# fabiocarrara/neural-ode-features

Measured on AMD Instinct MI355X. Metric: images/sec (fwd+adjoint) CIFAR-10 ODE-ResNet bs=128 at 1/2/4/8 GPU, higher is better.
Workload: dtype f32

## Files before the change

### neural-ode-features_amd/csrc/kernels_stem.hip

```cpp
#include "stem.h"

namespace node {

namespace {

typedef float f32x16 __attribute__((ext_vector_type(16)));
typedef __bf16 bf16x8 __attribute__((ext_vector_type(8)));
typedef __bf16 bf16x2 __attribute__((ext_vector_type(2)));
typedef float f32x2 __attribute__((ext_vector_type(2)));
typedef unsigned u32x4 __attribute__((ext_vector_type(4)));

__device__ __forceinline__ void split3(float x, bf16_t& h, bf16_t& m, bf16_t& l) {
  const __bf16 bh = (__bf16)x;
  const float r = x - (float)bh;
  const __bf16 bm = (__bf16)r;
  const float r2 = r - (float)bm;
  const __bf16 bl = (__bf16)r2;
  h = __builtin_bit_cast(bf16_t, bh);
  m = __builtin_bit_cast(bf16_t, bm);
  l = __builtin_bit_cast(bf16_t, bl);
}
__device__ __forceinline__ void split8(const float4& p, const float4& q, u32x4& hh, u32x4& mm, u32x4& ll) {
  const f32x2 v[4] = {{p.x, p.y}, {p.z, p.w}, {q.x, q.y}, {q.z, q.w}};
#pragma unroll
  for (int i = 0; i < 4; ++i) {
    const bf16x2 h = __builtin_convertvector(v[i], bf16x2);
    const f32x2 r = v[i] - __builtin_convertvector(h, f32x2);
    const bf16x2 m = __builtin_convertvector(r, bf16x2);
    const f32x2 r2 = r - __builtin_convertvector(m, f32x2);
    const bf16x2 l = __builtin_convertvector(r2, bf16x2);
    hh[i] = __builtin_bit_cast(unsigned, h);
    mm[i] = __builtin_bit_cast(unsigned, m);
    ll[i] = __builtin_bit_cast(unsigned, l);
  }
}
__device__ __forceinline__ float bf16_f(bf16_t v) { return __builtin_bit_cast(float, (unsigned)v << 16); }

typedef __attribute__((address_space(3))) void* lds_ptr_t;
typedef short s16x4 __attribute__((ext_vector_type(4)));
__device__ __forceinline__ int img_off(int row, int piece) { return row * 128 + ((piece ^ ((row >> 1) & 7)) << 4); }
__device__ __forceinline__ void glds16(const bf16_t* src, unsigned char* lds_dst) {
  __builtin_amdgcn_global_load_lds(reinterpret_cast<const void*>(src), (lds_ptr_t)lds_dst, 16, 0, 0);
}

__global__ __launch_bounds__(256) void k_stem_conv(const SConvArgs a) {
  constexpr int BM = 128, BN = 64;
  constexpr int A_PLANE = BM * 128, B_PLANE = BN * 128, A_BYTES = 3 * A_PLANE, BUF = A_BYTES + 3 * B_PLANE;
  extern __shared__ __align__(16) unsigned char smem[];
  int* out_off = reinterpret_cast<int*>(smem + 2 * BUF);
  const int t = threadIdx.x, lane = t & 63, wave = __builtin_amdgcn_readfirstlane(t >> 6);
  const int ntn = a.Cout / BN;
  int b = blockIdx.x;
  const int nblk = gridDim.x;
  if ((nblk & 7) == 0) b = (b & 7) * (nblk >> 3) + (b >> 3);
  const int ntn_all = (a.mode == 0 && a.w2 != nullptr) ? 2 * ntn : ntn;
  const int tile_m = b / ntn_all;
  int tile_n = b - tile_m * ntn_all;
  const bool shortcut_tile = tile_n >= ntn;
  if (shortcut_tile) tile_n -= ntn;
  int tile0 = 0, ch = a.cls_h[0], cw = a.cls_w[0], cpy = a.cls_py[0], cpx = a.cls_px[0], ntap = a.cls_ntap[0];
  unsigned long long taps = a.cls_taps[0];
#pragma unroll
  for (int c = 1; c < 4; ++c)
    if (c < a.nclass && tile_m >= a.cls_tile0[c]) {
      tile0 = a.cls_tile0[c]; ch = a.cls_h[c]; cw = a.cls_w[c]; cpy = a.cls_py[c]; cpx = a.cls_px[c]; ntap = a.cls_ntap[c];
      taps = a.cls_taps[c];
    }
  if (shortcut_tile) { ntap = 1; taps = (unsigned long long)((a.KH >> 1) * a.KW + (a.KW >> 1)); }
  const bf16_t* wsel = shortcut_tile ? a.w2 : a.w;
  const size_t wsel_plane = shortcut_tile ? a.w2_plane : a.w_plane;
  const int wtaps_one = shortcut_tile ? 1 : 0;
  const bool extra_k = a.mode == 1 && a.in2 != nullptr && cpy == 0 && cpx == 0 && a.step == 2;
  const int row0 = (tile_m - tile0) * BM;
  const int Mc = a.N * ch * cw;
  const int lrow = lane >> 3, lslot = lane & 7;
  int rn[4], roy[4], rox[4];
  bool rval[4];
#pragma unroll
  for (int j = 0; j < 4; ++j) {
    const int rl = 32 * wave + 8 * j + lrow, r = row0 + rl;
    rval[j] = r < Mc;
    rn[j] = roy[j] = rox[j] = 0;
    if (rval[j]) {
      rn[j] = r / (ch * cw);
      const int rem = r - rn[j] * ch * cw;
      const int cy = rem / cw;
      roy[j] = cy * a.step + cpy;
      rox[j] = (rem - cy * cw) * a.step + cpx;
    }
    if (lslot == 0) out_off[rl] = rval[j] ? (rn[j] * a.OH + roy[j]) * a.OW + rox[j] : -1;
  }
  const int ncc = a.Cin >> 6;
  const int nmain = ntap * ncc;
  const int nchunk = nmain + (extra_k ? ncc : 0);

  auto issue = [&](int q, int buf) {
    unsigned char* A = smem + buf * BUF;
    unsigned char* B = A + A_BYTES;
    const bool xk = q >= nmain;
    const int qq = xk ? q - nmain : q;
    const int ti = qq / ncc, c0 = (qq - ti * ncc) << 6;
    const int tap = xk ? 0 : (int)((taps >> (4 * ti)) & 15);
    const int ky = xk ? 0 : tap / a.KW, kx = xk ? 0 : tap - ky * a.KW;
    const int pad = xk ? 0 : a.pad;
    const bf16_t* in = xk ? a.in2 : a.in;
    const bf16_t* wq = xk ? a.w2 : wsel;
    const size_t wq_plane = xk ? a.w2_plane : wsel_plane;
    const int wtap = (xk || wtaps_one) ? 0 : tap;
#pragma unroll
    for (int j = 0; j < 4; ++j) {
      int iy, ix;
      bool ok = rval[j];
      if (a.mode == 0) {
        iy = (roy[j] << a.sshift) + ky - pad;
        ix = (rox[j] << a.sshift) + kx - pad;
      } else {
        const int ty = roy[j] + pad - ky, tx = rox[j] + pad - kx;
        ok = ok && ty >= 0 && tx >= 0;
        iy = ty >> a.sshift;
        ix = tx >> a.sshift;
      }
      ok = ok && (unsigned)iy < (unsigned)a.IH && (unsigned)ix < (unsigned)a.IW;
      const int irow = ok ? (rn[j] * a.IH + iy) * a.IW + ix : a.zero_row;
      const int rl = 32 * wave + 8 * j + lrow;
      const bf16_t* src = in + (size_t)irow * a.Cin + c0 + ((lslot ^ ((rl >> 1) & 7)) << 3);
#pragma unroll
      for (int p = 0; p < 3; ++p) glds16(src + p * a.in_plane, A + p * A_PLANE + (32 * wave + 8 * j) * 128);
    }
#pragma unroll
    for (int j = 0; j < 2; ++j) {
      const int col = 16 * wave + 8 * j + lrow;
      const bf16_t* ws = wq + ((size_t)wtap * a.Cout + tile_n * BN + col) * a.Cin + c0 + ((lslot ^ ((col >> 1) & 7)) << 3);
#pragma unroll
      for (int p = 0; p < 3; ++p) glds16(ws + p * wq_plane, B + p * B_PLANE + (16 * wave + 8 * j) * 128);
    }
  };

  f32x16 acc[2];
#pragma unroll
  for (int c = 0; c < 2; ++c)
#pragma unroll
    for (int i = 0; i < 16; ++i) acc[c][i] = 0.f;

  issue(0, 0);
  const int li = lane & 31, lg = lane >> 5;
  const int arow = 32 * wave + li;
  for (int q = 0; q < nchunk; ++q) {
    __syncthreads();
    if (q + 1 < nchunk) issue(q + 1, (q + 1) & 1);
    const unsigned char* A = smem + (q & 1) * BUF;
    const unsigned char* B = A + A_BYTES;
#pragma unroll
    for (int ks = 0; ks < 4; ++ks) {
      bf16x8 fa[3];
#pragma unroll
      for (int p = 0; p < 3; ++p)
        fa[p] = __builtin_bit_cast(bf16x8, *reinterpret_cast<const u32x4*>(A + p * A_PLANE + img_off(arow, 2 * ks + lg)));
#pragma unroll
      for (int c = 0; c < 2; ++c) {
        const int brow = 32 * c + li;
        bf16x8 fb[3];
#pragma unroll
        for (int p = 0; p < 3; ++p)
          fb[p] = __builtin_bit_cast(bf16x8, *reinterpret_cast<const u32x4*>(B + p * B_PLANE + img_off(brow, 2 * ks + lg)));
        acc[c] = __builtin_amdgcn_mfma_f32_32x32x16_bf16(fa[2], fb[0], acc[c], 0, 0, 0);
        acc[c] = __builtin_amdgcn_mfma_f32_32x32x16_bf16(fa[0], fb[2], acc[c], 0, 0, 0);
        acc[c] = __builtin_amdgcn_mfma_f32_32x32x16_bf16(fa[1], fb[1], acc[c], 0, 0, 0);
        acc[c] = __builtin_amdgcn_mfma_f32_32x32x16_bf16(fa[1], fb[0], acc[c], 0, 0, 0);
        acc[c] = __builtin_amdgcn_mfma_f32_32x32x16_bf16(fa[0], fb[1], acc[c], 0, 0, 0);
        acc[c] = __builtin_amdgcn_mfma_f32_32x32x16_bf16(fa[0], fb[0], acc[c], 0, 0, 0);
      }
    }
  }

#pragma unroll
  for (int c = 0; c < 2; ++c) {
    const int col = tile_n * BN + 32 * c + li;
    const float bv = a.bias ? a.bias[col] : 0.f;
#pragma unroll
    for (int i = 0; i < 16; ++i) {
      const int rl = 32 * wave + 8 * (i >> 2) + 4 * lg + (i & 3);
      const int off = out_off[rl];
      if (off < 0) continue;
      const size_t o = (size_t)off * a.Cout + col;
      if (shortcut_tile) { a.out2[o] = acc[c][i]; continue; }
      float v = acc[c][i] + bv;
      if (a.res) v += a.res[o];
      if (a.accumulate) v += a.out[o];
      a.out[o] = v;
    }
  }
}

template <int TG, bool EXTRA>
__global__ __launch_bounds__(256) void k_stem_wgrad(const SWgradArgs a) {
  constexpr int IMG = 3 * 16 * 128;
  constexpr int NIMG = 1 + TG + (EXTRA ? 1 : 0);
  constexpr int BUF = NIMG * IMG;
  extern __shared__ __align__(16) unsigned char smem[];
  const int t = threadIdx.x, lane = t & 63, wave = __builtin_amdgcn_readfirstlane(t >> 6);
  const int nct = a.Cin >> 6, npair = nct * (a.Cout >> 6);
  const int ngrp = TG == 3 ? 3 : 1;
  int bb = blockIdx.x;
  const int pair = bb % npair; bb /= npair;
  const int ky = bb % ngrp;
  const int split = bb / ngrp;
  const int cot = pair / nct, cit = pair - cot * nct;
  const bool extra = EXTRA && ky == 1;
  const int rows = a.N * a.OH * a.OW;
  const int rbeg = split * a.rows_per_split;
  const int rend = min(rbeg + a.rows_per_split, rows);
  const int nchunk = rbeg < rend ? (rend - rbeg + 15) >> 4 : 0;

  const int lrow = lane >> 3, lslot = lane & 7;
  int pn[2], py[2], px[2];
#pragma unroll
  for (int h = 0; h < 2; ++h) {
    const int r = rbeg + 8 * h + lrow;
    pn[h] = r / (a.OH * a.OW);
    const int rem = r - pn[h] * a.OH * a.OW;
    py[h] = rem / a.OW;
    px[h] = rem - py[h] * a.OW;
  }
  auto issue = [&](int q, int buf) {
    unsigned char* base = smem + buf * BUF;
    const int r0 = rbeg + 16 * q;
    constexpr int NINST = NIMG * 6;
#pragma unroll
    for (int ii = 0; ii < (NINST + 3) / 4; ++ii) {
      const int inst = wave + 4 * ii;
      if (inst >= NINST) break;
      const int im = inst / 6, part = (inst % 6) >> 1, h = inst & 1;
      if (EXTRA && !extra && im == NIMG - 1) continue;
      const int rl = 8 * h + lrow;
      const bool valid = r0 + rl < rend;
      const int sw = (lslot ^ ((rl >> 1) & 7)) << 3;
      const bf16_t* src;
      if (im == 0 || (EXTRA && im == NIMG - 1)) {
        const bf16_t* d = im == 0 ? a.dy3 : a.dy23;
        src = d + part * a.dy_plane + (size_t)(valid ? r0 + rl : a.dy_zero_row) * a.Cout + cot * 64 + sw;
      } else {
        const int kx = TG == 3 ? im - 1 : 0;
        const int iy = py[h] * a.stride - a.pad + (TG == 3 ? ky : 0), ix = px[h] * a.stride - a.pad + kx;
        const bool ok = valid && (unsigned)iy < (unsigned)a.IH && (unsigned)ix < (unsigned)a.IW;
        src = a.in + part * a.in_plane + (size_t)(ok ? (pn[h] * a.IH + iy) * a.IW + ix : a.zero_row) * a.Cin + cit * 64 + sw;
      }
      glds16(src, base + im * IMG + part * 2048 + h * 1024);
    }
#pragma unroll
    for (int h = 0; h < 2; ++h) {
      px[h] += 16;
      while (px[h] >= a.OW) { px[h] -= a.OW; py[h] += 1; }
      while (py[h] >= a.OH) { py[h] -= a.OH; pn[h] += 1; }
    }
  };

  constexpr int NA = TG + (EXTRA ? 1 : 0);
  f32x16 acc[NA];
#pragma unroll
  for (int j = 0; j < NA; ++j)
#pragma unroll
    for (int i = 0; i < 16; ++i) acc[j][i] = 0.f;

  const int cob = wave >> 1, cib = wave & 1;
  const int kg = lane >> 5, g16 = (lane >> 4) & 1, m = lane & 15, tq = m >> 2, tp = m & 3;
  auto frag = [&](const unsigned char* img, int part, int cb0) -> bf16x8 {
    const int piece = ((cb0 + 16 * g16) >> 3) + (tp >> 1), inb = (tp & 1) << 3;
    const int r0 = 8 * kg + tq, r1 = r0 + 4;
    const s16x4 lo = __builtin_amdgcn_ds_read_tr16_b64_v4i16((__attribute__((address_space(3))) s16x4*)(img + part * 2048 + img_off(r0, piece) + inb));
    const s16x4 hi = __builtin_amdgcn_ds_read_tr16_b64_v4i16((__attribute__((address_space(3))) s16x4*)(img + part * 2048 + img_off(r1, piece) + inb));
    typedef short s16x8 __attribute__((ext_vector_type(8)));
    const s16x8 v = {lo[0], lo[1], lo[2], lo[3], hi[0], hi[1], hi[2], hi[3]};
    return __builtin_bit_cast(bf16x8, v);
  };

  if (nchunk > 0) issue(0, 0);
  for (int q = 0; q < nchunk; ++q) {
    __syncthreads();
    if (q + 1 < nchunk) issue(q + 1, (q + 1) & 1);
    const unsigned char* base = smem + (q & 1) * BUF;
    bf16x8 fa[3];
#pragma unroll
    for (int p = 0; p < 3; ++p) fa[p] = frag(base, p, 32 * cob);
#pragma unroll
    for (int j = 0; j < TG; ++j) {
      bf16x8 fb[3];
#pragma unroll
      for (int p = 0; p < 3; ++p) fb[p] = frag(base + (1 + j) * IMG, p, 32 * cib);
      acc[j] = __builtin_amdgcn_mfma_f32_32x32x16_bf16(fa[2], fb[0], acc[j], 0, 0, 0);
      acc[j] = __builtin_amdgcn_mfma_f32_32x32x16_bf16(fa[0], fb[2], acc[j], 0, 0, 0);
      acc[j] = __builtin_amdgcn_mfma_f32_32x32x16_bf16(fa[1], fb[1], acc[j], 0, 0, 0);
      acc[j] = __builtin_amdgcn_mfma_f32_32x32x16_bf16(fa[1], fb[0], acc[j], 0, 0, 0);
      acc[j] = __builtin_amdgcn_mfma_f32_32x32x16_bf16(fa[0], fb[1], acc[j], 0, 0, 0);
      acc[j] = __builtin_amdgcn_mfma_f32_32x32x16_bf16(fa[0], fb[0], acc[j], 0, 0, 0);
      if (EXTRA && j == 1 && extra) {
        bf16x8 f2[3];
#pragma unroll
        for (int p = 0; p < 3; ++p) f2[p] = frag(base + (NIMG - 1) * IMG, p, 32 * cob);
        acc[TG] = __builtin_amdgcn_mfma_f32_32x32x16_bf16(f2[2], fb[0], acc[TG], 0, 0, 0);
        acc[TG] = __builtin_amdgcn_mfma_f32_32x32x16_bf16(f2[0], fb[2], acc[TG], 0, 0, 0);
        acc[TG] = __builtin_amdgcn_mfma_f32_32x32x16_bf16(f2[1], fb[1], acc[TG], 0, 0, 0);
        acc[TG] = __builtin_amdgcn_mfma_f32_32x32x16_bf16(f2[1], fb[0], acc[TG], 0, 0, 0);
        acc[TG] = __builtin_amdgcn_mfma_f32_32x32x16_bf16(f2[0], fb[1], acc[TG], 0, 0, 0);
        acc[TG] = __builtin_amdgcn_mfma_f32_32x32x16_bf16(f2[0], fb[0], acc[TG], 0, 0, 0);
      }
    }
  }
  const int li = lane & 31, hh = lane >> 5;
  const int taps_total = TG == 3 ? 9 : 1;
#pragma unroll
  for (int j = 0; j < NA; ++j) {
    if (j == TG && !extra) continue;
    float* dst = j < TG ? a.slab + ((size_t)split * taps_total + (TG == 3 ? ky * 3 + j : 0)) * a.Cout * a.Cin
                        : a.slab2 + (size_t)split * a.Cout * a.Cin;
#pragma unroll
    for (int i = 0; i < 16; ++i) {
      const int co = cot * 64 + 32 * cob + 8 * (i >> 2) + 4 * hh + (i & 3);
      dst[(size_t)co * a.Cin + cit * 64 + 32 * cib + li] = acc[j][i];
    }
  }
}

__global__ __launch_bounds__(256) void k_stem_conv0_fwd(const float* __restrict__ x, const float* __restrict__ w0t,
                                                        const float* __restrict__ bias, float* __restrict__ h0, int N, int Cin, int H,
                                                        int W) {
  const int t = threadIdx.x, lane = t & 63, wave = t >> 6, li = lane & 31, hh = lane >> 5;
  const int OH = H - 2, OW = W - 2, rows = N * OH * OW, K = 9 * Cin;
  const int row0 = (blockIdx.x * 4 + wave) * 32;
  if (row0 >= rows) return;
  const int r = row0 + li;
  const bool valid = r < rows;
  int base = 0;
  if (valid) {
    const int n = r / (OH * OW), rem = r - n * OH * OW, oy = rem / OW, ox = rem - oy * OW;
    base = (n * Cin * H + oy) * W + ox;
  }
  f32x16 acc0, acc1;
#pragma unroll
  for (int i = 0; i < 16; ++i) { acc0[i] = 0.f; acc1[i] = 0.f; }
  const int steps = (K + 1) >> 1;
  for (int s = 0; s < steps; ++s) {
    const int k = 2 * s + hh, kk = min(k, K - 1);
    const int ci = kk / 9, rem = kk - 9 * ci, ky = rem / 3, kx = rem - 3 * ky;
    const float av = valid ? x[base + (ci * H + ky) * W + kx] : 0.f;
    const float b0 = w0t[k * 64 + li], b1 = w0t[k * 64 + 32 + li];
    acc0 = __builtin_amdgcn_mfma_f32_32x32x2f32(av, b0, acc0, 0, 0, 0);
    acc1 = __builtin_amdgcn_mfma_f32_32x32x2f32(av, b1, acc1, 0, 0, 0);
  }
  const float bv0 = bias[li], bv1 = bias[32 + li];
#pragma unroll
  for (int i = 0; i < 16; ++i) {
    const int rr = row0 + 8 * (i >> 2) + 4 * hh + (i & 3);
    if (rr >= rows) continue;
    h0[(size_t)rr * 64 + li] = acc0[i] + bv0;
    h0[(size_t)rr * 64 + 32 + li] = acc1[i] + bv1;
  }
}

__global__ __launch_bounds__(256) void k_stem_conv0_wgrad(const float* __restrict__ x, const float* __restrict__ dh0,
                                                          float* __restrict__ slab, int N, int Cin, int H, int W, int rows_per_split) {
  __shared__ float red[2 * 16 * 64];
  const int t = threadIdx.x, lane = t & 63, wave = t >> 6, li = lane & 31, hh = lane >> 5;
  const int OH = H - 2, OW = W - 2, rows = N * OH * OW, K = 9 * Cin;
  const int per_wave = rows_per_split >> 2;
  const int rbeg = blockIdx.x * rows_per_split + wave * per_wave;
  const int rend = min(rbeg + per_wave, rows);
  int koff = 0;
  if (li < K) {
    const int ci = li / 9, rem = li - 9 * ci, ky = rem / 3;
    koff = (ci * H + ky) * W + (rem - 3 * ky);
  }
  int r = rbeg + hh;
  int n = 0, oy = 0, ox = 0;
  if (r < rows) {
    n = r / (OH * OW);
    const int rem = r - n * OH * OW;
    oy = rem / OW;
    ox = rem - oy * OW;
  }
  f32x16 acc0, acc1;
#pragma unroll
  for (int i = 0; i < 16; ++i) { acc0[i] = 0.f; acc1[i] = 0.f; }
  for (; r - hh < rend; r += 2) {
    const bool valid = r < rend;
    const float a0 = valid ? dh0[(size_t)r * 64 + li] : 0.f;
    const float a1 = valid ? dh0[(size_t)r * 64 + 32 + li] : 0.f;
    float bv = 0.f;
    if (valid) bv = li < K ? x[(n * Cin * H + oy) * W + ox + koff] : (li == K ? 1.f : 0.f);
    acc0 = __builtin_amdgcn_mfma_f32_32x32x2f32(a0, bv, acc0, 0, 0, 0);
    acc1 = __builtin_amdgcn_mfma_f32_32x32x2f32(a1, bv, acc1, 0, 0, 0);
    ox += 2;
    if (ox >= OW) {
      ox -= OW;
      oy += 1;
      if (oy >= OH) { oy = 0; n += 1; }
    }
  }
  for (int w = 1; w < 4; ++w) {
    if (wave == w) {
#pragma unroll
      for (int i = 0; i < 16; ++i) { red[i * 64 + lane] = acc0[i]; red[(16 + i) * 64 + lane] = acc1[i]; }
    }
    __syncthreads();
// ... 257 lines not shown
    const size_t of = ((size_t)tap * j.Cout + co) * j.Cin + ci, od = ((size_t)tap * j.Cin + ci) * j.Cout + co;
    j.wf[of] = h; j.wf[of + total] = m; j.wf[of + 2 * total] = l;
    j.wd[od] = h; j.wd[od + total] = m; j.wd[od + 2 * total] = l;
    return;
  }
  if (job == a.njobs) {
    if (a.w0t == nullptr || idx >= 28 * 64) return;
    const int k = (int)(idx / 64), co = (int)(idx % 64);
    a.w0t[idx] = k < a.k0 ? a.w0[co * a.k0 + k] : 0.f;
    return;
  }
  const int which = (int)(idx / 4096), e = (int)(idx % 4096);
  if (which >= a.nzero * 3) return;
  const int ten = which / 3, p = which - 3 * ten;
  if (e < a.zero_c[ten]) a.zero[ten][p * a.zero_plane[ten] + e] = 0;
}

__global__ __launch_bounds__(256) void k_stem_reduce(const SReduceArgs a) {
  __shared__ float part[4][64];
  int ji = 0;
  while (ji + 1 < a.njobs && blockIdx.x >= a.blk0[ji + 1]) ++ji;
  const SReduceJob& j = a.job[ji];
  const unsigned bx = blockIdx.x - a.blk0[ji];
  const int t = threadIdx.x;
  if (j.kind == 0) {
    const int co = bx / j.taps, tap = bx - co * j.taps;
    if (co >= j.Co) return;
    const size_t total = (size_t)j.taps * j.Co * j.Ci;
    const int cl = t & 63, sub = t >> 6;
    for (int c0 = 0; c0 < j.Ci; c0 += 64) {
      const float* src = j.slab + ((size_t)tap * j.Co + co) * j.Ci + c0 + cl;
      float s0 = 0.f, s1 = 0.f;
      int k = sub;
      for (; k + 28 < j.ns; k += 32) {
        float v[8];
#pragma unroll
        for (int q = 0; q < 8; ++q) v[q] = src[(size_t)(k + 4 * q) * total];
#pragma unroll
        for (int q = 0; q < 8; q += 2) { s0 += v[q]; s1 += v[q + 1]; }
      }
      for (; k + 4 < j.ns; k += 8) {
        s0 += src[(size_t)k * total];
        s1 += src[(size_t)(k + 4) * total];
      }
      if (k < j.ns) s0 += src[(size_t)k * total];
      part[sub][cl] = s0 + s1;
      __syncthreads();
      if (sub == 0) j.out[((size_t)co * j.Ci + c0 + cl) * j.taps + tap] = (part[0][cl] + part[1][cl]) + (part[2][cl] + part[3][cl]);
      __syncthreads();
    }
  } else {
    const size_t nout = j.kind == 1 ? (size_t)64 * 32 : (size_t)2 * j.Co;
    const int o = t & 31, g = t >> 5;
    const size_t idx = (size_t)bx * 32 + o;
    if ((size_t)bx * 32 >= nout) return;
    const bool on = idx < nout;
    const float* src = j.slab + (on ? idx : 0);
    float acc = 0.f;
    int k = g;
    for (; k + 56 < j.ns; k += 64) {
      float v[8];
#pragma unroll
      for (int q = 0; q < 8; ++q) v[q] = src[(size_t)(k + 8 * q) * nout];
      acc += ((v[0] + v[1]) + (v[2] + v[3])) + ((v[4] + v[5]) + (v[6] + v[7]));
    }
    for (; k < j.ns; k += 8) acc += src[(size_t)k * nout];
    part[g >> 1][(g & 1) * 32 + o] = acc;
    __syncthreads();
    if (g != 0 || !on) return;
    const float sum = ((part[0][o] + part[0][32 + o]) + (part[1][o] + part[1][32 + o])) + ((part[2][o] + part[2][32 + o]) + (part[3][o] + part[3][32 + o]));
    if (j.kind == 1) {
      const int co = (int)(idx >> 5), kk = (int)(idx & 31);
      if (kk < j.Ci) j.out[co * j.Ci + kk] = sum;
      else if (kk == j.Ci) j.out2[co] = sum;
    } else {
      if (idx < (size_t)j.Co) j.out[idx] = sum;
      else j.out2[idx - j.Co] = sum;
    }
  }
}

}

void launch_stem_conv(const SConvArgs& a, hipStream_t s) {
  const int mt = a.cls_tile0[a.nclass];
  static bool attr[MAX_DEVICES] = {};
  allow_full_lds(reinterpret_cast<const void*>(k_stem_conv), attr);
  const size_t lds = 2 * (3 * 128 * 128 + 3 * 64 * 128) + 512;
  const int ntn = (a.Cout / 64) * ((a.mode == 0 && a.w2 != nullptr) ? 2 : 1);
  hipLaunchKernelGGL(k_stem_conv, dim3(mt * ntn), dim3(256), lds, s, a);
}

void launch_stem_wgrad(const SWgradArgs& a, hipStream_t s) {
  const int taps = a.KH * a.KW;
  const int grid = (a.Cin / 64) * (a.Cout / 64) * (taps == 9 ? 3 : 1) * a.nsplit;
  const int nimg = 1 + (taps == 9 ? 3 : 1) + (a.dy23 ? 1 : 0);
  const size_t lds = (size_t)2 * nimg * 3 * 16 * 128;
#define STEM_WG(T, EX)                                                                   \
  {                                                                                       \
    static bool attr[MAX_DEVICES] = {};                                                   \
    allow_full_lds(reinterpret_cast<const void*>(k_stem_wgrad<T, EX>), attr);             \
    hipLaunchKernelGGL((k_stem_wgrad<T, EX>), dim3(grid), dim3(256), lds, s, a);           \
  }
  if (taps == 9 && a.dy23) STEM_WG(3, true)
  else if (taps == 9) STEM_WG(3, false)
  else STEM_WG(1, false)
#undef STEM_WG
}

void launch_stem_conv0_fwd(const float* x, const float* w0t, const float* bias, float* h0, int N, int Cin, int H, int W, hipStream_t s) {
  const int rows = N * (H - 2) * (W - 2);
  hipLaunchKernelGGL(k_stem_conv0_fwd, dim3((rows + 127) / 128), dim3(256), 0, s, x, w0t, bias, h0, N, Cin, H, W);
}
void launch_stem_conv0_wgrad(const float* x, const float* dh0, float* slab, int N, int Cin, int H, int W, int nsplit, int rows_per_split,
                             hipStream_t s) {
  hipLaunchKernelGGL(k_stem_conv0_wgrad, dim3(nsplit), dim3(256), 0, s, x, dh0, slab, N, Cin, H, W, rows_per_split);
}

int stem_gn_cb(int HW, int C, int cpg) {
  const size_t budget = 150 * 1024;
  int cb = 8;
  while (cb < cpg) cb *= 2;
  if (cb > C || cb > 128 || (size_t)HW * cb * 2 * sizeof(float) > budget) return 0;
  while (cb * 2 <= C && cb * 2 <= 128 && (size_t)HW * cb * 4 * sizeof(float) <= budget) cb *= 2;
  static const int cap = env_int("NODE_TUNE_STEM_GNCB", -1);
  while (cap > 0 && cb > cap && cb / 2 >= cpg && cb / 2 >= 8) cb /= 2;
  if (C % cb != 0 || cb % cpg != 0) return 0;
  return cb;
}
void launch_stem_gn_fwd(const SGnArgs& a, hipStream_t s) {
  static bool attr[MAX_DEVICES] = {};
  allow_full_lds(reinterpret_cast<const void*>(k_stem_gn_fwd), attr);
  hipLaunchKernelGGL(k_stem_gn_fwd, dim3(a.N * (a.C / a.CB)), dim3(256), ((size_t)a.HW * a.CB + 512) * sizeof(float), s, a);
}
void launch_stem_gn_bwd(const SGnArgs& a, hipStream_t s) {
  static bool attr[MAX_DEVICES] = {};
  allow_full_lds(reinterpret_cast<const void*>(k_stem_gn_bwd), attr);
  hipLaunchKernelGGL(k_stem_gn_bwd, dim3(a.N * (a.C / a.CB)), dim3(256), ((size_t)2 * a.HW * a.CB + 1024) * sizeof(float), s, a);
}

void launch_stem_prep(const SPrepArgs& a0, hipStream_t s) {
  SPrepArgs a = a0;
  unsigned at = 0;
  for (int i = 0; i < 6; ++i) {
    a.blk0[i] = at;
    if (i < a.njobs) at += (unsigned)(((size_t)a.job[i].taps * a.job[i].Cout * a.job[i].Cin + 255) / 256);
  }
  a.blk0[6] = at; at += (28 * 64 + 255) / 256;
  a.blk0[7] = at; at += (unsigned)(((size_t)a.nzero * 3 * 4096 + 255) / 256);
  a.blk0[8] = at;
  hipLaunchKernelGGL(k_stem_prep, dim3(at), dim3(256), 0, s, a);
}
void launch_stem_from_nchw(const float* src, float* dst_nhwc, bf16_t* dst3, size_t plane, int N, int C, int HW, hipStream_t s) {
  hipLaunchKernelGGL(k_stem_from_nchw, dim3(N * (C / 64) * ((HW + 63) / 64)), dim3(256), 0, s, src, dst_nhwc, dst3, plane, C, HW);
}
void launch_stem_split(const float* src, bf16_t* dst3, size_t plane, size_t n, hipStream_t s) {
  hipLaunchKernelGGL(k_stem_split, dim3((unsigned)((n / 8 + 255) / 256)), dim3(256), 0, s, src, dst3, plane, n / 8);
}
void launch_stem_to_nchw(const float* src_nhwc, float* dst, int N, int C, int HW, hipStream_t s) {
  hipLaunchKernelGGL(k_stem_to_nchw, dim3(N * (C / 64) * ((HW + 63) / 64)), dim3(256), 0, s, src_nhwc, dst, C, HW);
}
void launch_stem_reduce(const SReduceArgs& a0, hipStream_t s) {
  SReduceArgs a = a0;
  unsigned at = 0;
  for (int i = 0; i < a.njobs; ++i) {
    const SReduceJob& j = a.job[i];
    a.blk0[i] = at;
    at += (unsigned)(j.kind == 0 ? j.Co * j.taps : j.kind == 1 ? 64 : (2 * j.Co + 31) / 32);
  }
  a.blk0[a.njobs] = at;
  if (at == 0) return;
  hipLaunchKernelGGL(k_stem_reduce, dim3(at), dim3(256), 0, s, a);
}

}
```

Measured before the change: 28600.

## Pipeline stem conv and wgrad kernels with a multi-stage LDS ring

Replaces the double-buffered LDS staging in the stem conv and weight-gradient kernels with a ring of D+1 stages (D=3). Global-to-LDS loads for upcoming chunks are interleaved between MFMA pairs, and waits use explicit vmcnt counts instead of full __syncthreads. The conv kernel uses a narrower K chunk (32) and double-buffers its register fragments. The wgrad kernel is specialized per wave and per extra-branch, with incremental address stepping, and epilogue variants are templated on residual/accumulate. This targets load latency the old scheme left exposed. In exchange it uses more LDS per block, which may reduce occupancy, and adds inline-asm m0 handling that is fragile.

```diff
diff --git a/neural-ode-features_amd/csrc/kernels_stem.hip b/neural-ode-features_amd/csrc/kernels_stem.hip
--- a/neural-ode-features_amd/csrc/kernels_stem.hip
+++ b/neural-ode-features_amd/csrc/kernels_stem.hip
@@ -1,4 +1,5 @@
 #include "stem.h"
+#include <type_traits>
 
 namespace node {
 
@@ -38,16 +39,56 @@
 
 typedef __attribute__((address_space(3))) void* lds_ptr_t;
 typedef short s16x4 __attribute__((ext_vector_type(4)));
-__device__ __forceinline__ int img_off(int row, int piece) { return row * 128 + ((piece ^ ((row >> 1) & 7)) << 4); }
-__device__ __forceinline__ void glds16(const bf16_t* src, unsigned char* lds_dst) {
-  __builtin_amdgcn_global_load_lds(reinterpret_cast<const void*>(src), (lds_ptr_t)lds_dst, 16, 0, 0);
-}
-
+constexpr int STEM_RING_D = 3;
+template <int KC>
+__device__ __forceinline__ int img_off(int row, int piece) {
+  constexpr int PP = KC / 8, SH = KC == 64 ? 1 : 2;
+  return row * (2 * KC) + ((piece ^ ((row >> SH) & (PP - 1))) << 4);
+}
+__device__ __forceinline__ void glds16(const bf16_t* src, unsigned lds_dst) {
+  unsigned keep;
+  asm volatile("s_mov_b32 %0, m0\n\ts_mov_b32 m0, %2\n\ts_nop 0\n\tglobal_load_lds_dwordx4 %1, off\n\ts_mov_b32 m0, %0"
+               : "=&s"(keep) : "v"(src), "s"(lds_dst) : "memory");
+}
+template <int N>
+__device__ __forceinline__ void wait_vm() { asm volatile("s_waitcnt vmcnt(%0)" ::"n"(N) : "memory"); }
+template <int NP, int K>
+__device__ __forceinline__ void wait_stages(int ahead) {
+  if constexpr (K == 0) {
+    wait_vm<0>();
+  } else {
+    if (ahead >= K) wait_vm<K * NP>();
+    else wait_stages<NP, K - 1>(ahead);
+  }
+}
+template <class F>
+__device__ __forceinline__ void six_products(f32x16& acc, const bf16x8 (&x)[3], const bf16x8 (&y)[3], F&& between) {
+  acc = __builtin_amdgcn_mfma_f32_32x32x16_bf16(x[2], y[0], acc, 0, 0, 0);
+  acc = __builtin_amdgcn_mfma_f32_32x32x16_bf16(x[0], y[2], acc, 0, 0, 0);
+  between();
+  acc = __builtin_amdgcn_mfma_f32_32x32x16_bf16(x[1], y[1], acc, 0, 0, 0);
+  acc = __builtin_amdgcn_mfma_f32_32x32x16_bf16(x[1], y[0], acc, 0, 0, 0);
+  between();
+  acc = __builtin_amdgcn_mfma_f32_32x32x16_bf16(x[0], y[1], acc, 0, 0, 0);
+  acc = __builtin_amdgcn_mfma_f32_32x32x16_bf16(x[0], y[0], acc, 0, 0, 0);
+  between();
+}
+template <int NP, int D>
+__device__ __forceinline__ void ring_step(int q, int nq) {
+  wait_stages<NP, D - 1>(min(q + D - 1, nq - 1) - q);
+  asm volatile("s_waitcnt lgkmcnt(0)" ::: "memory");
+  __builtin_amdgcn_s_barrier();
+  asm volatile("" ::: "memory");
+}
+
+template <int KC, int D>
 __global__ __launch_bounds__(256) void k_stem_conv(const SConvArgs a) {
-  constexpr int BM = 128, BN = 64;
-  constexpr int A_PLANE = BM * 128, B_PLANE = BN * 128, A_BYTES = 3 * A_PLANE, BUF = A_BYTES + 3 * B_PLANE;
+  constexpr int BM = 128, BN = 64, NST = D + 1, KS = KC / 16;
+  constexpr int ROWB = 2 * KC, PP = KC / 8, RPI = 64 / PP, SH = KC == 64 ? 1 : 2;
+  constexpr int A_PLANE = BM * ROWB, B_PLANE = BN * ROWB, A_BYTES = 3 * A_PLANE, BUF = A_BYTES + 3 * B_PLANE;
+  constexpr int NJA = 32 / RPI, NJB = 16 / RPI, NP = 3 * (NJA + NJB);
   extern __shared__ __align__(16) unsigned char smem[];
-  int* out_off = reinterpret_cast<int*>(smem + 2 * BUF);
+  int* out_off = reinterpret_cast<int*>(smem + NST * BUF);
   const int t = threadIdx.x, lane = t & 63, wave = __builtin_amdgcn_readfirstlane(t >> 6);
   const int ntn = a.Cout / BN;
   int b = blockIdx.x;
@@ -73,12 +114,12 @@
   const bool extra_k = a.mode == 1 && a.in2 != nullptr && cpy == 0 && cpx == 0 && a.step == 2;
   const int row0 = (tile_m - tile0) * BM;
   const int Mc = a.N * ch * cw;
-  const int lrow = lane >> 3, lslot = lane & 7;
-  int rn[4], roy[4], rox[4];
-  bool rval[4];
-#pragma unroll
-  for (int j = 0; j < 4; ++j) {
-    const int rl = 32 * wave + 8 * j + lrow, r = row0 + rl;
+  const int lrow = lane / PP, lslot = lane & (PP - 1);
+  int rn[NJA], roy[NJA], rox[NJA];
+  bool rval[NJA];
+#pragma unroll
+  for (int j = 0; j < NJA; ++j) {
+    const int rl = 32 * wave + RPI * j + lrow, r = row0 + rl;
     rval[j] = r < Mc;
     rn[j] = roy[j] = rox[j] = 0;
     if (rval[j]) {
@@ -90,25 +131,26 @@
     }
     if (lslot == 0) out_off[rl] = rval[j] ? (rn[j] * a.OH + roy[j]) * a.OW + rox[j] : -1;
   }
-  const int ncc = a.Cin >> 6;
-  const int nmain = ntap * ncc;
-  const int nchunk = nmain + (extra_k ? ncc : 0);
-
-  auto issue = [&](int q, int buf) {
-    unsigned char* A = smem + buf * BUF;
-    unsigned char* B = A + A_BYTES;
-    const bool xk = q >= nmain;
-    const int qq = xk ? q - nmain : q;
-    const int ti = qq / ncc, c0 = (qq - ti * ncc) << 6;
-    const int tap = xk ? 0 : (int)((taps >> (4 * ti)) & 15);
-    const int ky = xk ? 0 : tap / a.KW, kx = xk ? 0 : tap - ky * a.KW;
+  const int ncc = a.Cin / KC;
+  const int nseg = ntap + (extra_k ? 1 : 0);
+  const int nchunk = nseg * ncc;
+
+  int i_seg = 0, i_cc = 0;
+  const bf16_t* asrc[NJA];
+  const bf16_t* bsrc[NJB];
+  size_t a_pl = 0, b_pl = 0;
+  auto set_segment = [&]() {
+    const bool xk = i_seg >= ntap;
+    const int tap = xk ? 0 : (int)((taps >> (4 * i_seg)) & 15);
+    const int ky = tap / a.KW, kx = tap - ky * a.KW;
     const int pad = xk ? 0 : a.pad;
     const bf16_t* in = xk ? a.in2 : a.in;
     const bf16_t* wq = xk ? a.w2 : wsel;
-    const size_t wq_plane = xk ? a.w2_plane : wsel_plane;
     const int wtap = (xk || wtaps_one) ? 0 : tap;
-#pragma unroll
-    for (int j = 0; j < 4; ++j) {
+    a_pl = a.in_plane;
+    b_pl = xk ? a.w2_plane : wsel_plane;
+#pragma unroll
+    for (int j = 0; j < NJA; ++j) {
       int iy, ix;
       bool ok = rval[j];
       if (a.mode == 0) {
@@ -122,19 +164,29 @@
       }
       ok = ok && (unsigned)iy < (unsigned)a.IH && (unsigned)ix < (unsigned)a.IW;
       const int irow = ok ? (rn[j] * a.IH + iy) * a.IW + ix : a.zero_row;
-      const int rl = 32 * wave + 8 * j + lrow;
-      const bf16_t* src = in + (size_t)irow * a.Cin + c0 + ((lslot ^ ((rl >> 1) & 7)) << 3);
-#pragma unroll
-      for (int p = 0; p < 3; ++p) glds16(src + p * a.in_plane, A + p * A_PLANE + (32 * wave + 8 * j) * 128);
-    }
-#pragma unroll
-    for (int j = 0; j < 2; ++j) {
-      const int col = 16 * wave + 8 * j + lrow;
-      const bf16_t* ws = wq + ((size_t)wtap * a.Cout + tile_n * BN + col) * a.Cin + c0 + ((lslot ^ ((col >> 1) & 7)) << 3);
-#pragma unroll
-      for (int p = 0; p < 3; ++p) glds16(ws + p * wq_plane, B + p * B_PLANE + (16 * wave + 8 * j) * 128);
+      const int rl = 32 * wave + RPI * j + lrow;
+      asrc[j] = in + (size_t)irow * a.Cin + ((lslot ^ ((rl >> SH) & (PP - 1))) << 3);
+    }
+#pragma unroll
+    for (int j = 0; j < NJB; ++j) {
+      const int col = 16 * wave + RPI * j + lrow;
+      bsrc[j] = wq + ((size_t)wtap * a.Cout + tile_n * BN + col) * a.Cin + ((lslot ^ ((col >> SH) & (PP - 1))) << 3);
     }
   };
+  const unsigned lds0 = (unsigned)(size_t)(lds_ptr_t)smem;
+  auto piece = [&](int k, int stage) {
+    const bool isb = k >= 3 * NJA;
+    const int kk = isb ? k - 3 * NJA : k, j = kk / 3, p = kk - 3 * j;
+    const int c0 = i_cc * KC;
+    if (!isb) glds16(asrc[j] + p * a_pl + c0, lds0 + stage * BUF + 32 * wave * ROWB + p * A_PLANE + j * RPI * ROWB);
+    else glds16(bsrc[j] + p * b_pl + c0, lds0 + stage * BUF + A_BYTES + 16 * wave * ROWB + p * B_PLANE + j * RPI * ROWB);
+  };
+  auto next_chunk = [&]() {
+    if (++i_cc == ncc) {
+      i_cc = 0;
+      if (++i_seg < nseg) set_segment();
+    }
+  };
 
   f32x16 acc[2];
 #pragma unroll
@@ -142,63 +194,114 @@
 #pragma unroll
     for (int i = 0; i < 16; ++i) acc[c][i] = 0.f;
 
-  issue(0, 0);
+  set_segment();
+#pragma unroll
+  for (int q = 0; q < D; ++q)
+    if (q < nchunk) {
+#pragma unroll
+      for (int k = 0; k < NP; ++k) piece(k, q);
+      next_chunk();
+    }
   const int li = lane & 31, lg = lane >> 5;
   const int arow = 32 * wave + li;
-  for (int q = 0; q < nchunk; ++q) {
-    __syncthreads();
-    if (q + 1 < nchunk) issue(q + 1, (q + 1) & 1);
-    const unsigned char* A = smem + (q & 1) * BUF;
+  int st_read = 0, st_fill = D;
+  auto step = [&](int q, auto fill) {
+    constexpr bool FILL = decltype(fill)::value;
+    ring_step<NP, D>(q, nchunk);
+    const unsigned char* A = smem + st_read * BUF;
     const unsigned char* B = A + A_BYTES;
-#pragma unroll
-    for (int ks = 0; ks < 4; ++ks) {
-      bf16x8 fa[3];
+    bf16x8 fa[2][3], fb[2][2][3];
+    auto fetch = [&](int ks, int s) {
 #pragma unroll
       for (int p = 0; p < 3; ++p)
-        fa[p] = __builtin_bit_cast(bf16x8, *reinterpret_cast<const u32x4*>(A + p * A_PLANE + img_off(arow, 2 * ks + lg)));
-#pragma unroll
-      for (int c = 0; c < 2; ++c) {
-        const int brow = 32 * c + li;
-        bf16x8 fb[3];
+        fa[s][p] = __builtin_bit_cast(bf16x8, *reinterpret_cast<const u32x4*>(A + p * A_PLANE + img_off<KC>(arow, 2 * ks + lg)));
+#pragma unroll
+      for (int c = 0; c < 2; ++c)
 #pragma unroll
         for (int p = 0; p < 3; ++p)
-          fb[p] = __builtin_bit_cast(bf16x8, *reinterpret_cast<const u32x4*>(B + p * B_PLANE + img_off(brow, 2 * ks + lg)));
-        acc[c] = __builtin_amdgcn_mfma_f32_32x32x16_bf16(fa[2], fb[0], acc[c], 0, 0, 0);
-        acc[c] = __builtin_amdgcn_mfma_f32_32x32x16_bf16(fa[0], fb[2], acc[c], 0, 0, 0);
-        acc[c] = __builtin_amdgcn_mfma_f32_32x32x16_bf16(fa[1], fb[1], acc[c], 0, 0, 0);
-        acc[c] = __builtin_amdgcn_mfma_f32_32x32x16_bf16(fa[1], fb[0], acc[c], 0, 0, 0);
-        acc[c] = __builtin_amdgcn_mfma_f32_32x32x16_bf16(fa[0], fb[1], acc[c], 0, 0, 0);
-        acc[c] = __builtin_amdgcn_mfma_f32_32x32x16_bf16(fa[0], fb[0], acc[c], 0, 0, 0);
+          fb[s][c][p] = __builtin_bit_cast(bf16x8, *reinterpret_cast<const u32x4*>(B + p * B_PLANE + img_off<KC>(32 * c + li, 2 * ks + lg)));
+    };
+    int pk = 0;
+    auto between = [&]() {
+      if constexpr (FILL) {
+        if (pk < NP) piece(pk, st_fill);
+        ++pk;
+        __builtin_amdgcn_sched_barrier(0);
       }
-    }
-  }
-
-#pragma unroll
-  for (int c = 0; c < 2; ++c) {
-    const int col = tile_n * BN + 32 * c + li;
-    const float bv = a.bias ? a.bias[col] : 0.f;
-#pragma unroll
-    for (int i = 0; i < 16; ++i) {
-      const int rl = 32 * wave + 8 * (i >> 2) + 4 * lg + (i & 3);
-      const int off = out_off[rl];
-      if (off < 0) continue;
-      const size_t o = (size_t)off * a.Cout + col;
-      if (shortcut_tile) { a.out2[o] = acc[c][i]; continue; }
-      float v = acc[c][i] + bv;
-      if (a.res) v += a.res[o];
-      if (a.accumulate) v += a.out[o];
-      a.out[o] = v;
-    }
-  }
-}
-
-template <int TG, bool EXTRA>
-__global__ __launch_bounds__(256) void k_stem_wgrad(const SWgradArgs a) {
+    };
+    fetch(0, 0);
+#pragma unroll
+    for (int ks = 0; ks < KS; ++ks) {
+      const int s = ks & 1;
+      if (ks + 1 < KS) fetch(ks + 1, s ^ 1);
+      if constexpr (FILL) __builtin_amdgcn_sched_barrier(0);
+#pragma unroll
+      for (int c = 0; c < 2; ++c) six_products(acc[c], fa[s], fb[s][c], between);
+    }
+    static_assert(NP <= 6 * KS, "a chunk's pieces go between its MFMA pairs");
+    if constexpr (FILL) next_chunk();
+    st_read = st_read + 1 == NST ? 0 : st_read + 1;
+    st_fill = st_fill + 1 == NST ? 0 : st_fill + 1;
+  };
+  int q = 0;
+  for (; q + D < nchunk; ++q) step(q, std::true_type());
+  for (; q < nchunk; ++q) step(q, std::false_type());
+
+  int off[16];
+#pragma unroll
+  for (int i = 0; i < 16; ++i) off[i] = out_off[32 * wave + 8 * (i >> 2) + 4 * lg + (i & 3)];
+  const int col0 = tile_n * BN + li;
+  if (shortcut_tile) {
+#pragma unroll
+    for (int c = 0; c < 2; ++c)
+#pragma unroll
+      for (int i = 0; i < 16; ++i)
+        if (off[i] >= 0) a.out2[(size_t)off[i] * a.Cout + col0 + 32 * c] = acc[c][i];
+    return;
+  }
+  const float bv[2] = {a.bias ? a.bias[col0] : 0.f, a.bias ? a.bias[col0 + 32] : 0.f};
+  auto finish = [&](auto has_res, auto has_out) {
+    constexpr bool RES = decltype(has_res)::value, OUT = decltype(has_out)::value;
+    float r[2][16], o[2][16];
+#pragma unroll
+    for (int c = 0; c < 2; ++c)
+#pragma unroll
+      for (int i = 0; i < 16; ++i) {
+        const size_t e = (size_t)max(off[i], 0) * a.Cout + col0 + 32 * c;
+        if constexpr (RES) r[c][i] = a.res[e];
+        if constexpr (OUT) o[c][i] = a.out[e];
+      }
+#pragma unroll
+    for (int c = 0; c < 2; ++c)
+#pragma unroll
+      for (int i = 0; i < 16; ++i) {
+        float v = acc[c][i] + bv[c];
+        if constexpr (RES) v += r[c][i];
+        if constexpr (OUT) v += o[c][i];
+        if (off[i] >= 0) a.out[(size_t)off[i] * a.Cout + col0 + 32 * c] = v;
+      }
+  };
+  typedef std::true_type yes;
+  typedef std::false_type no;
+  if (a.res) {
+    if (a.accumulate) finish(yes(), yes());
+    else finish(yes(), no());
+  } else {
+    if (a.accumulate) finish(no(), yes());
+    else finish(no(), no());
+  }
+}
+
+template <int TG, bool EX, int D, int W>
+__device__ __forceinline__ void stem_wgrad_wave(const SWgradArgs& a, unsigned char* smem) {
+  constexpr int NST = D + 1;
   constexpr int IMG = 3 * 16 * 128;
-  constexpr int NIMG = 1 + TG + (EXTRA ? 1 : 0);
+  constexpr int NIMG = 1 + TG + (EX ? 1 : 0);
   constexpr int BUF = NIMG * IMG;
-  extern __shared__ __align__(16) unsigned char smem[];
-  const int t = threadIdx.x, lane = t & 63, wave = __builtin_amdgcn_readfirstlane(t >> 6);
+  constexpr int NINST = NIMG * 6;
+  constexpr int NP = (NINST - W + 3) / 4;
+  constexpr int H = W & 1;
+  const int lane = threadIdx.x & 63;
   const int nct = a.Cin >> 6, npair = nct * (a.Cout >> 6);
   const int ngrp = TG == 3 ? 3 : 1;
   int bb = blockIdx.x;
@@ -206,111 +309,124 @@
   const int ky = bb % ngrp;
   const int split = bb / ngrp;
   const int cot = pair / nct, cit = pair - cot * nct;
-  const bool extra = EXTRA && ky == 1;
   const int rows = a.N * a.OH * a.OW;
   const int rbeg = split * a.rows_per_split;
   const int rend = min(rbeg + a.rows_per_split, rows);
   const int nchunk = rbeg < rend ? (rend - rbeg + 15) >> 4 : 0;
 
-  const int lrow = lane >> 3, lslot = lane & 7;
-  int pn[2], py[2], px[2];
-#pragma unroll
-  for (int h = 0; h < 2; ++h) {
-    const int r = rbeg + 8 * h + lrow;
-    pn[h] = r / (a.OH * a.OW);
-    const int rem = r - pn[h] * a.OH * a.OW;
-    py[h] = rem / a.OW;
-    px[h] = rem - py[h] * a.OW;
-  }
-  auto issue = [&](int q, int buf) {
-    unsigned char* base = smem + buf * BUF;
-    const int r0 = rbeg + 16 * q;
-    constexpr int NINST = NIMG * 6;
-#pragma unroll
-    for (int ii = 0; ii < (NINST + 3) / 4; ++ii) {
-      const int inst = wave + 4 * ii;
-      if (inst >= NINST) break;
-      const int im = inst / 6, part = (inst % 6) >> 1, h = inst & 1;
-      if (EXTRA && !extra && im == NIMG - 1) continue;
-      const int rl = 8 * h + lrow;
-      const bool valid = r0 + rl < rend;
-      const int sw = (lslot ^ ((rl >> 1) & 7)) << 3;
-      const bf16_t* src;
-      if (im == 0 || (EXTRA && im == NIMG - 1)) {
-        const bf16_t* d = im == 0 ? a.dy3 : a.dy23;
-        src = d + part * a.dy_plane + (size_t)(valid ? r0 + rl : a.dy_zero_row) * a.Cout + cot * 64 + sw;
-      } else {
-        const int kx = TG == 3 ? im - 1 : 0;
-        const int iy = py[h] * a.stride - a.pad + (TG == 3 ? ky : 0), ix = px[h] * a.stride - a.pad + kx;
-        const bool ok = valid && (unsigned)iy < (unsigned)a.IH && (unsigned)ix < (unsigned)a.IW;
-        src = a.in + part * a.in_plane + (size_t)(ok ? (pn[h] * a.IH + iy) * a.IW + ix : a.zero_row) * a.Cin + cit * 64 + sw;
-      }
-      glds16(src, base + im * IMG + part * 2048 + h * 1024);
-    }
-#pragma unroll
-    for (int h = 0; h < 2; ++h) {
-      px[h] += 16;
-      while (px[h] >= a.OW) { px[h] -= a.OW; py[h] += 1; }
-      while (py[h] >= a.OH) { py[h] -= a.OH; pn[h] += 1; }
-    }
+  const int rl = 8 * H + (lane >> 3);
+  const int sw = ((lane & 7) ^ ((rl >> 1) & 7)) << 3;
+  const int ohw = a.OH * a.OW;
+  const int an = 16 / ohw, ay = (16 - an * ohw) / a.OW, ax = 16 - an * ohw - ay * a.OW;
+  const int d_irow = (an * a.IH + ay * a.stride) * a.IW + ax * a.stride;
+  const int cx_irow = (a.IW - a.OW) * a.stride, cy_irow = (a.IH - a.OH * a.stride) * a.IW;
+  int r = rbeg + rl;
+  int py, px, irow;
+  {
+    const int pn = r / ohw, rem = r - pn * ohw;
+    py = rem / a.OW;
+    px = rem - py * a.OW;
+    irow = (pn * a.IH + py * a.stride - a.pad + (TG == 3 ? ky : 0)) * a.IW + px * a.stride - a.pad;
+  }
+  const bf16_t* dyb = a.dy3 + cot * 64 + sw;
+  const bf16_t* dy2b = EX ? a.dy23 + cot * 64 + sw : nullptr;
+  const bf16_t* inb = a.in + cit * 64 + sw;
+  const unsigned lds0 = (unsigned)(size_t)(lds_ptr_t)smem;
+  size_t dyo, ino[TG];
+  auto sources = [&]() {
+    const bool valid = r < rend;
+    const int iy = py * a.stride - a.pad + (TG == 3 ? ky : 0), ix0 = px * a.stride - a.pad;
+    const bool oky = valid && (unsigned)iy < (unsigned)a.IH;
+    dyo = (size_t)(valid ? r : a.dy_zero_row) * a.Cout;
+#pragma unroll
+    for (int kx = 0; kx < TG; ++kx) {
+      const bool ok = oky && (unsigned)(ix0 + kx) < (unsigned)a.IW;
+      ino[kx] = (size_t)(ok ? irow + kx : a.zero_row) * a.Cin;
+    }
+    r += 16;
+    px += ax; py += ay; irow += d_irow;
+    if (px >= a.OW) { px -= a.OW; py += 1; irow += cx_irow; }
+    if (py >= a.OH) { py -= a.OH; irow += cy_irow; }
   };
-
-  constexpr int NA = TG + (EXTRA ? 1 : 0);
+  auto piece = [&](int ii, int stage) {
+    const int inst = W + 4 * ii, im = inst / 6, part = (inst % 6) >> 1;
+    const int kx = im >= 1 && im <= TG ? im - 1 : 0;
+    const bf16_t* src = im == 0 ? dyb + part * a.dy_plane + dyo
+                      : im > TG ? dy2b + part * a.dy_plane + dyo
+                                : inb + part * a.in_plane + ino[kx];
+    glds16(src, lds0 + stage * BUF + im * IMG + part * 2048 + H * 1024);
+  };
+
+  constexpr int NA = TG + (EX ? 1 : 0);
   f32x16 acc[NA];
 #pragma unroll
   for (int j = 0; j < NA; ++j)
 #pragma unroll
     for (int i = 0; i < 16; ++i) acc[j][i] = 0.f;
 
-  const int cob = wave >> 1, cib = wave & 1;
+  constexpr int cob = W >> 1, cib = W & 1;
   const int kg = lane >> 5, g16 = (lane >> 4) & 1, m = lane & 15, tq = m >> 2, tp = m & 3;
   auto frag = [&](const unsigned char* img, int part, int cb0) -> bf16x8 {
-    const int piece = ((cb0 + 16 * g16) >> 3) + (tp >> 1), inb = (tp & 1) << 3;
+    const int piece = ((cb0 + 16 * g16) >> 3) + (tp >> 1), inb8 = (tp & 1) << 3;
     const int r0 = 8 * kg + tq, r1 = r0 + 4;
-    const s16x4 lo = __builtin_amdgcn_ds_read_tr16_b64_v4i16((__attribute__((address_space(3))) s16x4*)(img + part * 2048 + img_off(r0, piece) + inb));
-    const s16x4 hi = __builtin_amdgcn_ds_read_tr16_b64_v4i16((__attribute__((address_space(3))) s16x4*)(img + part * 2048 + img_off(r1, piece) + inb));
+    const s16x4 lo = __builtin_amdgcn_ds_read_tr16_b64_v4i16((__attribute__((address_space(3))) s16x4*)(img + part * 2048 + img_off<64>(r0, piece) + inb8));
+    const s16x4 hi = __builtin_amdgcn_ds_read_tr16_b64_v4i16((__attribute__((address_space(3))) s16x4*)(img + part * 2048 + img_off<64>(r1, piece) + inb8));
     typedef short s16x8 __attribute__((ext_vector_type(8)));
     const s16x8 v = {lo[0], lo[1], lo[2], lo[3], hi[0], hi[1], hi[2], hi[3]};
     return __builtin_bit_cast(bf16x8, v);
   };
 
-  if (nchunk > 0) issue(0, 0);
-  for (int q = 0; q < nchunk; ++q) {
-    __syncthreads();
-    if (q + 1 < nchunk) issue(q + 1, (q + 1) & 1);
-    const unsigned char* base = smem + (q & 1) * BUF;
-    bf16x8 fa[3];
+#pragma unroll
+  for (int q = 0; q < D; ++q)
+    if (q < nchunk) {
+      sources();
+#pragma unroll
+      for (int ii = 0; ii < NP; ++ii) piece(ii, q);
+    }
+  int st_read = 0, st_fill = D;
+  auto step = [&](int q, auto fill) {
+    constexpr bool FILL = decltype(fill)::value;
+    ring_step<NP, D>(q, nchunk);
+    if constexpr (FILL) sources();
+    const unsigned char* base = smem + st_read * BUF;
+    bf16x8 fa[3], fb[TG][3], f2[3];
 #pragma unroll
     for (int p = 0; p < 3; ++p) fa[p] = frag(base, p, 32 * cob);
 #pragma unroll
+    for (int j = 0; j < TG; ++j)
+#pragma unroll
+      for (int p = 0; p < 3; ++p) fb[j][p] = frag(base + (1 + j) * IMG, p, 32 * cib);
+    if constexpr (EX) {
+#pragma unroll
+      for (int p = 0; p < 3; ++p) f2[p] = frag(base + (NIMG - 1) * IMG, p, 32 * cob);
+    }
+    int pk = 0;
+    auto between = [&]() {
+      if constexpr (FILL) {
+        if (pk < NP) piece(pk, st_fill);
+        ++pk;
+        __builtin_amdgcn_sched_barrier(0);
+      }
+    };
+    if constexpr (FILL) __builtin_amdgcn_sched_barrier(0);
+#pragma unroll
     for (int j = 0; j < TG; ++j) {
-      bf16x8 fb[3];
-#pragma unroll
-      for (int p = 0; p < 3; ++p) fb[p] = frag(base + (1 + j) * IMG, p, 32 * cib);
-      acc[j] = __builtin_amdgcn_mfma_f32_32x32x16_bf16(fa[2], fb[0], acc[j], 0, 0, 0);
-      acc[j] = __builtin_amdgcn_mfma_f32_32x32x16_bf16(fa[0], fb[2], acc[j], 0, 0, 0);
-      acc[j] = __builtin_amdgcn_mfma_f32_32x32x16_bf16(fa[1], fb[1], acc[j], 0, 0, 0);
-      acc[j] = __builtin_amdgcn_mfma_f32_32x32x16_bf16(fa[1], fb[0], acc[j], 0, 0, 0);
-      acc[j] = __builtin_amdgcn_mfma_f32_32x32x16_bf16(fa[0], fb[1], acc[j], 0, 0, 0);
-      acc[j] = __builtin_amdgcn_mfma_f32_32x32x16_bf16(fa[0], fb[0], acc[j], 0, 0, 0);
-      if (EXTRA && j == 1 && extra) {
-        bf16x8 f2[3];
-#pragma unroll
-        for (int p = 0; p < 3; ++p) f2[p] = frag(base + (NIMG - 1) * IMG, p, 32 * cob);
-        acc[TG] = __builtin_amdgcn_mfma_f32_32x32x16_bf16(f2[2], fb[0], acc[TG], 0, 0, 0);
-        acc[TG] = __builtin_amdgcn_mfma_f32_32x32x16_bf16(f2[0], fb[2], acc[TG], 0, 0, 0);
-        acc[TG] = __builtin_amdgcn_mfma_f32_32x32x16_bf16(f2[1], fb[1], acc[TG], 0, 0, 0);
-        acc[TG] = __builtin_amdgcn_mfma_f32_32x32x16_bf16(f2[1], fb[0], acc[TG], 0, 0, 0);
-        acc[TG] = __builtin_amdgcn_mfma_f32_32x32x16_bf16(f2[0], fb[1], acc[TG], 0, 0, 0);
-        acc[TG] = __builtin_amdgcn_mfma_f32_32x32x16_bf16(f2[0], fb[0], acc[TG], 0, 0, 0);
+      six_products(acc[j], fa, fb[j], between);
+      if constexpr (EX) {
+        if (j == 1) six_products(acc[TG], f2, fb[j], between);
       }
     }
-  }
+    static_assert(NP <= 3 * NA, "a chunk's pieces go between its MFMA pairs");
+    st_read = st_read + 1 == NST ? 0 : st_read + 1;
+    st_fill = st_fill + 1 == NST ? 0 : st_fill + 1;
+  };
+  int q = 0;
+  for (; q + D < nchunk; ++q) step(q, std::true_type());
+  for (; q < nchunk; ++q) step(q, std::false_type());
   const int li = lane & 31, hh = lane >> 5;
   const int taps_total = TG == 3 ? 9 : 1;
 #pragma unroll
   for (int j = 0; j < NA; ++j) {
-    if (j == TG && !extra) continue;
     float* dst = j < TG ? a.slab + ((size_t)split * taps_total + (TG == 3 ? ky * 3 + j : 0)) * a.Cout * a.Cin
                         : a.slab2 + (size_t)split * a.Cout * a.Cin;
 #pragma unroll
@@ -319,6 +435,28 @@
       dst[(size_t)co * a.Cin + cit * 64 + 32 * cib + li] = acc[j][i];
     }
   }
+}
+
+template <int TG, bool EX, int D>
+__device__ __forceinline__ void stem_wgrad_waves(const SWgradArgs& a, unsigned char* smem, int wave) {
+  if (wave == 0) stem_wgrad_wave<TG, EX, D, 0>(a, smem);
+  else if (wave == 1) stem_wgrad_wave<TG, EX, D, 1>(a, smem);
+  else if (wave == 2) stem_wgrad_wave<TG, EX, D, 2>(a, smem);
+  else stem_wgrad_wave<TG, EX, D, 3>(a, smem);
+}
+
+template <int TG, bool EXTRA, int D>
+__global__ __launch_bounds__(256) void k_stem_wgrad(const SWgradArgs a) {
+  extern __shared__ __align__(16) unsigned char smem[];
+  const int wave = __builtin_amdgcn_readfirstlane(threadIdx.x >> 6);
+  if constexpr (EXTRA) {
+    const int npair = (a.Cin >> 6) * (a.Cout >> 6);
+    if ((blockIdx.x / npair) % 3 == 1) {
+      stem_wgrad_waves<TG, true, D>(a, smem, wave);
+      return;
+    }
+  }
+  stem_wgrad_waves<TG, false, D>(a, smem, wave);
 }
 
 __global__ __launch_bounds__(256) void k_stem_conv0_fwd(const float* __restrict__ x, const float* __restrict__ w0t,
@@ -742,29 +880,43 @@
 
 }
 
+static bool stem_ring() { return env_int("NODE_TUNE_STEM_RING", 1) != 0; }
+
 void launch_stem_conv(const SConvArgs& a, hipStream_t s) {
   const int mt = a.cls_tile0[a.nclass];
-  static bool attr[MAX_DEVICES] = {};
-  allow_full_lds(reinterpret_cast<const void*>(k_stem_conv), attr);
-  const size_t lds = 2 * (3 * 128 * 128 + 3 * 64 * 128) + 512;
   const int ntn = (a.Cout / 64) * ((a.mode == 0 && a.w2 != nullptr) ? 2 : 1);
-  hipLaunchKernelGGL(k_stem_conv, dim3(mt * ntn), dim3(256), lds, s, a);
+#define STEM_CONV(KC, D)                                                                  \
+  {                                                                                       \
+    static bool attr[MAX_DEVICES] = {};                                                   \
+    allow_full_lds(reinterpret_cast<const void*>(k_stem_conv<KC, D>), attr);              \
+    const size_t lds = (size_t)(D + 1) * (3 * 128 + 3 * 64) * 2 * KC + 512;               \
+    hipLaunchKernelGGL((k_stem_conv<KC, D>), dim3(mt * ntn), dim3(256), lds, s, a);        \
+  }
+  if (stem_ring()) STEM_CONV(32, STEM_RING_D)
+  else STEM_CONV(64, 1)
+#undef STEM_CONV
 }
 
 void launch_stem_wgrad(const SWgradArgs& a, hipStream_t s) {
   const int taps = a.KH * a.KW;
   const int grid = (a.Cin / 64) * (a.Cout / 64) * (taps == 9 ? 3 : 1) * a.nsplit;
   const int nimg = 1 + (taps == 9 ? 3 : 1) + (a.dy23 ? 1 : 0);
-  const size_t lds = (size_t)2 * nimg * 3 * 16 * 128;
-#define STEM_WG(T, EX)                                                                   \
+#define STEM_WG(T, EX, D)                                                                \
   {                                                                                       \
     static bool attr[MAX_DEVICES] = {};                                                   \
-    allow_full_lds(reinterpret_cast<const void*>(k_stem_wgrad<T, EX>), attr);             \
-    hipLaunchKernelGGL((k_stem_wgrad<T, EX>), dim3(grid), dim3(256), lds, s, a);           \
-  }
-  if (taps == 9 && a.dy23) STEM_WG(3, true)
-  else if (taps == 9) STEM_WG(3, false)
-  else STEM_WG(1, false)
+    allow_full_lds(reinterpret_cast<const void*>(k_stem_wgrad<T, EX, D>), attr);          \
+    const size_t lds = (size_t)(D + 1) * nimg * 3 * 16 * 128;                             \
+    hipLaunchKernelGGL((k_stem_wgrad<T, EX, D>), dim3(grid), dim3(256), lds, s, a);        \
+  }
+  if (stem_ring()) {
+    if (taps == 9 && a.dy23) STEM_WG(3, true, STEM_RING_D)
+    else if (taps == 9) STEM_WG(3, false, STEM_RING_D)
+    else STEM_WG(1, false, STEM_RING_D)
+  } else {
+    if (taps == 9 && a.dy23) STEM_WG(3, true, 1)
+    else if (taps == 9) STEM_WG(3, false, 1)
+    else STEM_WG(1, false, 1)
+  }
 #undef STEM_WG
 }
 
```

After: 29580 (median of 6 runs). 3.4% higher.
